# 5l1v3r1/PBS

Measured on AMD Instinct MI355X. Metric: co-run slowdown (%) vs solo + aggregate throughput, 4-tenant mix at 1/2/4/8 GPU, higher is better.
Workload: dtype bf16

## Files before the change

### csrc/hip/common.hpp

```cpp
#pragma once
#include <hip/hip_runtime.h>

#include <cstdint>
#include <cstdio>
#include <cstdlib>

namespace gpbs_hip {

constexpr int kXcds = 8;
constexpr int kMaxTenants = 64;
constexpr int kNumPmc = 4;
constexpr uint32_t kNoOwner = 0xFFFFFFFFu;
constexpr uint32_t kSplitBit = 0x80000000u;
constexpr uint32_t kOwnerMask = 0x7FFFFFFFu;

typedef __bf16 bf16x8 __attribute__((ext_vector_type(8)));
typedef float f32x4 __attribute__((ext_vector_type(4)));
typedef float f32x16 __attribute__((ext_vector_type(16)));
typedef unsigned int u32x4 __attribute__((ext_vector_type(4)));
typedef unsigned int u32x2 __attribute__((ext_vector_type(2)));
typedef unsigned short u16;
typedef unsigned int u32;
typedef unsigned long long u64;

__device__ __forceinline__ float bfl(u32 w) { return __uint_as_float(w << 16); }
__device__ __forceinline__ float bfh(u32 w) { return __uint_as_float(w & 0xffff0000u); }
__device__ __forceinline__ u32 pack2(float lo, float hi) {
  return (u32)__builtin_bit_cast(u16, (__bf16)lo) | ((u32)__builtin_bit_cast(u16, (__bf16)hi) << 16);
}

constexpr int kCtx = 4;
struct alignas(64) PartTable {
  u32 epoch;
  u32 flags;
  u32 hold;
  u32 pad0;
  union {
    u32 owner[kXcds * kCtx];
    u64 pair[kXcds][2];
  };
  u32 pad[12];
};
static_assert(sizeof(PartTable) == 192, "partition table layout");

struct alignas(64) WorkQueue {
  u32 next;
  u32 done;
  u32 exited;
  u32 stopped;
  u32 xnext[kXcds];
  u32 pad[4];
};

__device__ __forceinline__ void finish(WorkQueue* q, u32* status, u32 total) {
  if (threadIdx.x == 0) {
    asm volatile("s_waitcnt vmcnt(0)" ::: "memory");
    const u32 old = atomicAdd(&q->exited, 1u);
    if (old == gridDim.x - 1) {
      const u32 d = __hip_atomic_load(&q->done, __ATOMIC_RELAXED, __HIP_MEMORY_SCOPE_AGENT);
      if (status) __hip_atomic_store(status, d | 0x80000000u, __ATOMIC_RELAXED, __HIP_MEMORY_SCOPE_SYSTEM);
      __hip_atomic_store(&q->exited, 0u, __ATOMIC_RELAXED, __HIP_MEMORY_SCOPE_AGENT);
      __hip_atomic_store(&q->stopped, 0u, __ATOMIC_RELAXED, __HIP_MEMORY_SCOPE_AGENT);
      if (d >= total) {
        __hip_atomic_store(&q->next, 0u, __ATOMIC_RELAXED, __HIP_MEMORY_SCOPE_AGENT);
        __hip_atomic_store(&q->done, 0u, __ATOMIC_RELAXED, __HIP_MEMORY_SCOPE_AGENT);
#pragma unroll
        for (int x = 0; x < kXcds; ++x) __hip_atomic_store(&q->xnext[x], 0u, __ATOMIC_RELAXED, __HIP_MEMORY_SCOPE_AGENT);
      }
    }
  }
}


enum GateMode : u32 {
  GATE_NONE = 0, GATE_TABLE = 1, GATE_PARK = 2, GATE_DEVTABLE = 4, GATE_SPATIAL = 8,
  GATE_WAVEPRIO = 16,
  GATE_SE = 32,
  GATE_HOLD = 64,
};
constexpr u32 kParkSpins = 100;
constexpr u32 kHoldSpins = 256;

#define HIPCHECK(x)                                                                              \
  do {                                                                                           \
    hipError_t _e = (x);                                                                         \
    if (_e != hipSuccess) {                                                                      \
      fprintf(stderr, "[gpbs-hip] %s:%d %s -> %s\n", __FILE__, __LINE__, #x, hipGetErrorString(_e)); \
      return -(int)_e - 1000;                                                                    \
    }                                                                                            \
  } while (0)

__device__ __forceinline__ u32 xcc_id() {
  return __builtin_amdgcn_s_getreg((3 << 11) | (0 << 6) | 20);
}

__device__ __forceinline__ u32 hw_id() { return __builtin_amdgcn_s_getreg((31 << 11) | (0 << 6) | 4); }

__device__ __forceinline__ u32 cu_half() { return (hw_id() >> 14) & 1u; }

__device__ __forceinline__ u32 se_id() { return (hw_id() >> 13) & 3u; }

__device__ __forceinline__ u32 load_sys(const u32* p) {
  return __hip_atomic_load(p, __ATOMIC_RELAXED, __HIP_MEMORY_SCOPE_SYSTEM);
}

__device__ __forceinline__ void hold_wait(const PartTable* t, u32 mode) {
  if (!(mode & GATE_HOLD)) return;
  for (u32 k = 0; k < kHoldSpins; ++k) {
    const u32 h = (mode & GATE_DEVTABLE) ? __hip_atomic_load(&t->hold, __ATOMIC_RELAXED, __HIP_MEMORY_SCOPE_AGENT)
                                         : __hip_atomic_load(&t->hold, __ATOMIC_RELAXED, __HIP_MEMORY_SCOPE_SYSTEM);
    if (!h) return;
    __builtin_amdgcn_s_sleep(32);
  }
}

__device__ __forceinline__ bool owns(const PartTable* t, u32 mode, u32 me, u32 xcc) {
  if ((mode & 3) == GATE_NONE) return true;
  if (mode & GATE_SE) {
    const u32 se = se_id();
    const u32* w = t->owner + kCtx * (xcc & 7) + se;
    const u32 o = (mode & GATE_DEVTABLE) ? __hip_atomic_load(w, __ATOMIC_RELAXED, __HIP_MEMORY_SCOPE_AGENT)
                                         : __hip_atomic_load(w, __ATOMIC_RELAXED, __HIP_MEMORY_SCOPE_SYSTEM);
    return (o & kOwnerMask) == me;
  }
  const u64* q = t->pair[xcc & 7];
  const u64 p01 = (mode & GATE_DEVTABLE) ? __hip_atomic_load(q, __ATOMIC_RELAXED, __HIP_MEMORY_SCOPE_AGENT)
                                         : __hip_atomic_load(q, __ATOMIC_RELAXED, __HIP_MEMORY_SCOPE_SYSTEM);
  const u32 w0 = (u32)p01, w1 = (u32)(p01 >> 32);
  const bool h0 = (w0 & kOwnerMask) == me, h1 = (w1 & kOwnerMask) == me;
  if (!(mode & GATE_SPATIAL) || (h0 && h1)) {
    if (h0 || h1) return true;
    const u64 p23 = (mode & GATE_DEVTABLE) ? __hip_atomic_load(q + 1, __ATOMIC_RELAXED, __HIP_MEMORY_SCOPE_AGENT)
                                           : __hip_atomic_load(q + 1, __ATOMIC_RELAXED, __HIP_MEMORY_SCOPE_SYSTEM);
    return (u32)p23 == me || (u32)(p23 >> 32) == me;
  }
  if (h0) return !(w0 & kSplitBit) || cu_half() == 0;
  if (h1) return !(w1 & kSplitBit) || cu_half() == 1;
  return false;
}

__device__ __forceinline__ void count(u64* cnt, u32 me, u32 xcc, u64 inst, u64 cyc, u64 refs, u64 miss) {
  if (!cnt) return;
  u64* c = cnt + ((size_t)me * kXcds + (xcc & 7)) * kNumPmc;
  if (inst) __hip_atomic_fetch_add(c + 0, inst, __ATOMIC_RELAXED, __HIP_MEMORY_SCOPE_SYSTEM);
  if (cyc) __hip_atomic_fetch_add(c + 1, cyc, __ATOMIC_RELAXED, __HIP_MEMORY_SCOPE_SYSTEM);
  if (refs) __hip_atomic_fetch_add(c + 2, refs, __ATOMIC_RELAXED, __HIP_MEMORY_SCOPE_SYSTEM);
  if (miss) __hip_atomic_fetch_add(c + 3, miss, __ATOMIC_RELAXED, __HIP_MEMORY_SCOPE_SYSTEM);
}

__device__ __forceinline__ int grab_unit(WorkQueue* q, const PartTable* table, u32 mode, u32 me, u32 xcc,
                                         int* s_slot, u32 total) {
  if (threadIdx.x == 0) {
    int u = -1;
    hold_wait(table, mode);
    for (u32 spins = 0;; ++spins) {
      if (owns(table, mode, me, xcc)) {
        const u32 t = atomicAdd(&q->next, 1u);
        u = t < total ? (int)t : -1;
        break;
      }
      if ((mode & 3) != GATE_PARK || spins >= kParkSpins ||
          __hip_atomic_load(&q->next, __ATOMIC_RELAXED, __HIP_MEMORY_SCOPE_AGENT) >= total) {
        atomicAdd(&q->stopped, 1u);
        break;
      }
#pragma unroll
      for (int k = 0; k < 6; ++k) __builtin_amdgcn_s_sleep(127);
    }
    *s_slot = u;
  }
  __syncthreads();
  int u = *s_slot;
  __syncthreads();
  return u;
}


__device__ __forceinline__ void count_unit(u64* cnt, u32 me, u32 xcc, u64 inst, u64* t_last, u64 refs, u64 miss,
                                           WorkQueue* q) {
  if (threadIdx.x != 0) return;
  const u64 t = __builtin_amdgcn_s_memtime();
  count(cnt, me, xcc, inst, t - *t_last, refs, miss);
  *t_last = t;
  atomicAdd(&q->done, 1u);
}

}
```

### csrc/hip/fp8_gemm_kernels.hip

```cpp
#include "common.hpp"

namespace gpbs_fp8g {

using namespace gpbs_hip;

typedef int i32x8 __attribute__((ext_vector_type(8)));
typedef __attribute__((address_space(3))) char lds_t;

constexpr int FBM = 128, FBN = 128, FBK = 128, FNT = 256;
constexpr int kTile = FBM * FBK;
constexpr int kLds = 2 * 2 * kTile;
constexpr int kOne = 0x7f7f7f7f;

__device__ __forceinline__ void glds16(const void* g, lds_t* l) {
  __builtin_amdgcn_global_load_lds(g, (__attribute__((address_space(3))) void*)l, 16, 0, 0);
}

__device__ __forceinline__ u16 f2bf(float x) { return __builtin_bit_cast(u16, (__bf16)x); }

template <int BSHUF>
__global__ __launch_bounds__(FNT, 2) void k_gemm_fp8_tn(const unsigned char* __restrict__ A,
                                                        const float* __restrict__ sa,
                                                        const unsigned char* __restrict__ B,
                                                        const float* __restrict__ sb, u16* __restrict__ C, int M,
                                                        int N, int K, WorkQueue* q, const PartTable* table, u32 mode,
                                                        u32 me, u64* cnt, u32 inst_per_tile, u32 refs_per_tile,
                                                        u32 miss_per_tile, u32* status) {
  __shared__ __attribute__((aligned(16))) char smem[kLds + 16];
  lds_t* lds = (lds_t*)smem;
  int* s_slot = (int*)(smem + kLds);
  const u32 xcc = xcc_id();
  u64 t_last = __builtin_amdgcn_s_memtime();
  const int tid = threadIdx.x, lane = tid & 63, wid = tid >> 6;
  const int wr = wid >> 1, wc = wid & 1;
  const int tiles_m = (M + FBM - 1) / FBM, tiles_n = N / FBN, ntiles = tiles_m * tiles_n;
  const int nk = K / FBK;
  constexpr int GROUP_M = 8;

  int srow[4], schunk[4];
#pragma unroll
  for (int j = 0; j < 4; ++j) {
    srow[j] = 8 * (wid * 4 + j) + (lane >> 3);
    schunk[j] = (lane & 7) ^ (srow[j] & 7);
  }
  const int l16 = lane & 15, lq = lane >> 4;

  for (;;) {
    const int t = grab_unit(q, table, mode, me, xcc, s_slot, (u32)ntiles);
    if (t < 0) break;
    const int in_group = GROUP_M * tiles_n;
    const int g = t / in_group;
    const int first_m = g * GROUP_M;
    const int gsz = min(tiles_m - first_m, GROUP_M);
    const int tm = first_m + (t % in_group) % gsz;
    const int tn = (t % in_group) / gsz;

    size_t aoff[4], boff[4];
    int bstep;
#pragma unroll
    for (int j = 0; j < 4; ++j) {
      const int ra = min(tm * FBM + srow[j], M - 1);
      aoff[j] = (size_t)ra * K + schunk[j] * 16;
      if (BSHUF) {
        const int p = wid * 4 + j;
        boff[j] = (size_t)(tn * (FBN / 16) + (p >> 1)) * (K >> 8) * 4096 + (p & 1) * 1024 + lane * 16;
      } else {
        boff[j] = (size_t)(tn * FBN + srow[j]) * K + schunk[j] * 16;
      }
    }
    bstep = BSHUF ? 2048 : FBK;

    f32x4 acc[4][4];
#pragma unroll
    for (int i = 0; i < 4; ++i)
#pragma unroll
      for (int j = 0; j < 4; ++j) acc[i][j] = f32x4{0.f, 0.f, 0.f, 0.f};

    auto stage = [&](int buf, int kt) {
      lds_t* la = lds + buf * (2 * kTile);
      lds_t* lb = la + kTile;
#pragma unroll
      for (int j = 0; j < 4; ++j) {
        const int c = wid * 4 + j;
        glds16(A + aoff[j] + (size_t)kt * FBK, la + c * 1024);
        glds16(B + boff[j] + (size_t)kt * bstep, lb + c * 1024);
      }
    };
    auto frag = [&](const lds_t* img, int r0) -> i32x8 {
      const int r = r0 + l16;
      const lds_t* row = img + r * 128;
      const u32x4 lo = *(const __attribute__((address_space(3))) u32x4*)(row + (((2 * lq) ^ (r & 7)) << 4));
      const u32x4 hi = *(const __attribute__((address_space(3))) u32x4*)(row + (((2 * lq + 1) ^ (r & 7)) << 4));
      return i32x8{(int)lo[0], (int)lo[1], (int)lo[2], (int)lo[3], (int)hi[0], (int)hi[1], (int)hi[2], (int)hi[3]};
    };
    auto frag_shuf = [&](const lds_t* img, int r0) -> i32x8 {
      const lds_t* p = img + ((r0 >> 4) * 2 + (lq >> 1)) * 1024 + (lq & 1) * 512 + l16 * 16;
      const u32x4 lo = *(const __attribute__((address_space(3))) u32x4*)p;
      const u32x4 hi = *(const __attribute__((address_space(3))) u32x4*)(p + 256);
      return i32x8{(int)lo[0], (int)lo[1], (int)lo[2], (int)lo[3], (int)hi[0], (int)hi[1], (int)hi[2], (int)hi[3]};
    };

    stage(0, 0);
    asm volatile("s_waitcnt vmcnt(0)" ::: "memory");
    __syncthreads();
    int cur = 0;
    for (int kt = 0; kt < nk; ++kt) {
      if (kt + 1 < nk) stage(cur ^ 1, kt + 1);
      const lds_t* la = lds + cur * (2 * kTile);
      const lds_t* lb = la + kTile;
      i32x8 a[4], b[4];
#pragma unroll
      for (int i = 0; i < 4; ++i) {
        a[i] = frag(la, wr * 64 + i * 16);
        b[i] = BSHUF ? frag_shuf(lb, wc * 64 + i * 16) : frag(lb, wc * 64 + i * 16);
      }
#pragma unroll
      for (int i = 0; i < 4; ++i)
#pragma unroll
        for (int j = 0; j < 4; ++j)
          acc[i][j] = __builtin_amdgcn_mfma_scale_f32_16x16x128_f8f6f4(a[i], b[j], acc[i][j], 0, 0, 0, kOne, 0, kOne);
      asm volatile("s_waitcnt vmcnt(0)" ::: "memory");
      __syncthreads();
      cur ^= 1;
    }
#pragma unroll
    for (int j = 0; j < 4; ++j) {
      const int n = tn * FBN + wc * 64 + j * 16 + l16;
      const float wsc = sb[n];
#pragma unroll
      for (int i = 0; i < 4; ++i) {
        const int m = tm * FBM + wr * 64 + i * 16 + lq * 4;
#pragma unroll
        for (int r = 0; r < 4; ++r)
          if (m + r < M) C[(size_t)(m + r) * N + n] = f2bf((acc[i][j][r] * sa[m + r]) * wsc);
      }
    }
    count_unit(cnt, me, xcc, inst_per_tile, &t_last, refs_per_tile, miss_per_tile, q);
  }
  finish(q, status, (u32)ntiles);
}

}

using namespace gpbs_fp8g;

extern "C" {

int gpbs_hip_gemm_fp8_units(int M, int N) {
  if (M <= 0 || N <= 0 || N % FBN) return 0;
  return ((M + FBM - 1) / FBM) * (N / FBN);
}

int gpbs_hip_gemm_fp8(const void* Aq, const float* sa, const void* Bq, const float* sb, void* C, int M, int N, int K,
                      int b_shuffled, void* q, const void* table, unsigned mode, unsigned me, void* cnt, void* status,
                      int grid, hipStream_t s) {
  if (M <= 0 || N <= 0 || K <= 0 || N % FBN || K % FBK || (b_shuffled && K % 256)) return -22;
  const int ntiles = ((M + FBM - 1) / FBM) * (N / FBN);
  if (grid <= 0) grid = 256 * 2;
  if (grid > ntiles) grid = ntiles;
  const u32 inst = (u32)((K / FBK) * (64 + 32 + 64) + 64);
  const u32 refs = (u32)(((u64)(FBM + FBN) * K) / 128);
  const u32 miss = (u32)((((u64)M + N) * K / 128) / ntiles + (u64)FBM * FBN * 2 / 128);
  auto kern = b_shuffled ? k_gemm_fp8_tn<1> : k_gemm_fp8_tn<0>;
  hipLaunchKernelGGL(kern, dim3(grid), dim3(FNT), 0, s, (const unsigned char*)Aq, sa, (const unsigned char*)Bq, sb,
                     (u16*)C, M, N, K, (WorkQueue*)q, (const PartTable*)table, mode, me, (u64*)cnt, inst, refs, miss,
                     (u32*)status);
  return hipGetLastError() == hipSuccess ? 0 : -5;
}

}
```

### csrc/hip/tenant_kernels.hip

```cpp
#include "common.hpp"

namespace gpbs_hip {


__device__ __forceinline__ int grab_unit_x(WorkQueue* q, const PartTable* table, u32 mode, u32 me, u32 xcc,
                                           int* s_slot, u32 total) {
  if (threadIdx.x == 0) {
    int u = -1;
    hold_wait(table, mode);
    const u32 per = (total + kXcds - 1) / kXcds;
    for (u32 spins = 0;; ++spins) {
      if (owns(table, mode, me, xcc)) {
        for (u32 k = 0; k < (u32)kXcds; ++k) {
          const u32 r = (xcc + k) & (kXcds - 1);
          const u32 lo = r * per, hi = min(lo + per, total);
          if (lo >= hi) continue;
          if (__hip_atomic_load(&q->xnext[r], __ATOMIC_RELAXED, __HIP_MEMORY_SCOPE_AGENT) >= hi - lo) continue;
          const u32 t = atomicAdd(&q->xnext[r], 1u);
          if (t < hi - lo) {
            u = (int)(lo + t);
            atomicAdd(&q->next, 1u);
            break;
          }
        }
        break;
      }
      if ((mode & 3) != GATE_PARK || spins >= kParkSpins ||
          __hip_atomic_load(&q->next, __ATOMIC_RELAXED, __HIP_MEMORY_SCOPE_AGENT) >= total) {
        atomicAdd(&q->stopped, 1u);
        break;
      }
#pragma unroll
      for (int k = 0; k < 6; ++k) __builtin_amdgcn_s_sleep(127);
    }
    *s_slot = u;
  }
  __syncthreads();
  int u = *s_slot;
  __syncthreads();
  return u;
}


__device__ __forceinline__ u16 f2bf(float x) { return __builtin_bit_cast(u16, (__bf16)x); }
__device__ __forceinline__ float bf2f(u16 x) { return __uint_as_float(((u32)x) << 16); }

constexpr int GBM = 128, GBN = 128, GBK = 64, GNT = 256;
constexpr int kGemmLds = 2 * 2 * GBM * GBK * 2;

typedef __attribute__((address_space(3))) char lds_t;

__device__ __forceinline__ void glds16(const void* g, lds_t* l) {
  __builtin_amdgcn_global_load_lds(g, (__attribute__((address_space(3))) void*)l, 16, 0, 0);
}

__global__ __launch_bounds__(GNT, 2) void k_gemm_bf16_tn(const u16* __restrict__ A, const u16* __restrict__ Bt,
                                                         u16* __restrict__ C, int M, int N, int K, WorkQueue* q,
                                                         const PartTable* table, u32 mode, u32 me, u64* cnt,
                                                         u32 inst_per_tile, u32 refs_per_tile, u32 miss_per_tile,
                                                         u32* status) {
  __shared__ __attribute__((aligned(16))) char smem[kGemmLds + 16];
  lds_t* lds = (lds_t*)smem;
  int* s_slot = (int*)(smem + kGemmLds);
  const u32 xcc = xcc_id();
  u64 t_last = __builtin_amdgcn_s_memtime();
  const int tid = threadIdx.x, lane = tid & 63, wid = tid >> 6;
  const int wr = wid >> 1, wc = wid & 1;
  const int tiles_m = M / GBM, tiles_n = N / GBN, ntiles = tiles_m * tiles_n;
  const int nk = K / GBK;
  constexpr int GROUP_M = 8;

  int srow[4], scol[4];
#pragma unroll
  for (int j = 0; j < 4; ++j) {
    const int c = wid * 4 + j;
    srow[j] = 8 * c + (lane >> 3);
    scol[j] = (((lane & 7) ^ (srow[j] & 7)) * 8);
  }

  for (;;) {
    const int t = grab_unit(q, table, mode, me, xcc, s_slot, (u32)ntiles);
    if (t < 0) break;
    const int in_group = GROUP_M * tiles_n;
    const int g = t / in_group;
    const int first_m = g * GROUP_M;
    const int gsz = min(tiles_m - first_m, GROUP_M);
    const int tm = first_m + (t % in_group) % gsz;
    const int tn = (t % in_group) / gsz;
    const u16* Ab = A + (size_t)tm * GBM * K;
    const u16* Bb = Bt + (size_t)tn * GBN * K;

    f32x4 acc[4][4];
#pragma unroll
    for (int i = 0; i < 4; ++i)
#pragma unroll
      for (int j = 0; j < 4; ++j) acc[i][j] = f32x4{0.f, 0.f, 0.f, 0.f};

    auto stage = [&](int buf, int kt) {
      lds_t* la = lds + buf * (2 * GBM * GBK * 2);
      lds_t* lb = la + GBM * GBK * 2;
#pragma unroll
      for (int j = 0; j < 4; ++j) {
        const int c = wid * 4 + j;
        glds16(Ab + (size_t)srow[j] * K + kt * GBK + scol[j], la + c * 1024);
        glds16(Bb + (size_t)srow[j] * K + kt * GBK + scol[j], lb + c * 1024);
      }
    };

    stage(0, 0);
    asm volatile("s_waitcnt vmcnt(0)" ::: "memory");
    __syncthreads();
    int cur = 0;
    for (int kt = 0; kt < nk; ++kt) {
      if (kt + 1 < nk) stage(cur ^ 1, kt + 1);
      const lds_t* la = lds + cur * (2 * GBM * GBK * 2);
      const lds_t* lb = la + GBM * GBK * 2;
#pragma unroll
      for (int s = 0; s < 2; ++s) {
        bf16x8 a[4], b[4];
        const int chunk = s * 4 + (lane >> 4);
#pragma unroll
        for (int i = 0; i < 4; ++i) {
          const int ra = wr * 64 + i * 16 + (lane & 15);
          a[i] = *(const __attribute__((address_space(3))) bf16x8*)(la + ra * 128 + ((chunk ^ (ra & 7)) << 4));
          const int rb = wc * 64 + i * 16 + (lane & 15);
          b[i] = *(const __attribute__((address_space(3))) bf16x8*)(lb + rb * 128 + ((chunk ^ (rb & 7)) << 4));
        }
#pragma unroll
        for (int i = 0; i < 4; ++i)
#pragma unroll
          for (int j = 0; j < 4; ++j) acc[i][j] = __builtin_amdgcn_mfma_f32_16x16x32_bf16(a[i], b[j], acc[i][j], 0, 0, 0);
      }
      asm volatile("s_waitcnt vmcnt(0)" ::: "memory");
      __syncthreads();
      cur ^= 1;
    }
#pragma unroll
    for (int i = 0; i < 4; ++i)
#pragma unroll
      for (int j = 0; j < 4; ++j) {
        const int m = tm * GBM + wr * 64 + i * 16 + (lane >> 4) * 4;
        const int n = tn * GBN + wc * 64 + j * 16 + (lane & 15);
#pragma unroll
        for (int r = 0; r < 4; ++r) C[(size_t)(m + r) * N + n] = f2bf(acc[i][j][r]);
      }
    count_unit(cnt, me, xcc, inst_per_tile, &t_last, refs_per_tile, miss_per_tile, q);
  }
  finish(q, status, (u32)ntiles);
}

constexpr int G2_BM = 256, G2_BK = 64, G2_NT = 512;
constexpr u32 kGemmXRange = 1u << 16;
constexpr u32 kGemmBlock2D = 1u << 17;
constexpr u32 kGemmStatic = 1u << 18;
constexpr int kGemmOptsLive = 1 | 8 | 1 << 23;
constexpr int kGemmOptsShipped = 256 | 8192 | 65536 | 131072;
static int g_gemm_opts = 8;
constexpr int kG2Half = 128 * 128;
constexpr int kG2Buf = 4 * kG2Half;
constexpr int kG2Lds = 2 * kG2Buf;

__device__ __forceinline__ int g2_swz(int r) { return (r >> 1) & 7; }

__global__ __launch_bounds__(G2_NT, 1) void k_gemm256_bf16_tn(const u16* __restrict__ A, const u16* __restrict__ Bt,
                                                             u16* __restrict__ C, int M, int N, int K, WorkQueue* q,
                                                             const PartTable* table, u32 mode, u32 me, u64* cnt,
                                                             u32 inst_per_tile, u32 refs_per_tile, u32 miss_per_tile,
                                                             u32* status) {
  __shared__ __attribute__((aligned(16))) char smem[kG2Lds + 16];
  lds_t* lds = (lds_t*)smem;
  int* s_slot = (int*)(smem + kG2Lds);
  const u32 xcc = xcc_id();
  u64 t_last = __builtin_amdgcn_s_memtime();
  const int tid = threadIdx.x, lane = tid & 63, wid = tid >> 6;
  const int wu = __builtin_amdgcn_readfirstlane(wid);
  const int wr = wu >> 2, wc = wu & 3;
  const int tiles_m = M / G2_BM, tiles_n = N / G2_BM, ntiles = tiles_m * tiles_n;
  const int nt = K / G2_BK;
  int soff[2];
#pragma unroll
  for (int j = 0; j < 2; ++j) {
    const int row = 8 * (2 * wid + j) + (lane >> 3);
    soff[j] = row * K + (((lane & 7) ^ g2_swz(row)) * 8);
  }
  int soffa[4];
#pragma unroll
  for (int j = 0; j < 4; ++j) {
    const int row = 8 * (4 * (wid & 3) + j) + (lane >> 3);
    soffa[j] = row * K + (((lane & 7) ^ g2_swz(row)) * 8);
  }
  const int l16 = lane & 15, lq = lane >> 4;
  const int bh = wc >> 1, bc = (wc & 1) * 64;
  int units_seen = 0;

  for (;;) {
    const int tile = (mode & kGemmStatic) ? (units_seen ? -1 : (int)blockIdx.x)
                     : (mode & kGemmXRange) ? grab_unit_x(q, table, mode, me, xcc, s_slot, (u32)ntiles)
                                            : grab_unit(q, table, mode, me, xcc, s_slot, (u32)ntiles);
    if (tile < 0) break;
    int tm = tile / tiles_n, tn = tile % tiles_n;
    if ((mode & kGemmBlock2D) && (tiles_m & 3) == 0 && (tiles_n & 1) == 0 && ntiles % kXcds == 0) {
      const int per = ntiles / kXcds;
      const int bm = tiles_m / 4, bn = tiles_n / 2;
      const int g = (mode & kGemmXRange) ? tile / per : tile % kXcds;
      const int jj = (mode & kGemmXRange) ? tile % per : tile / kXcds;
      tm = (g >> 1) * bm + jj / bn;
      tn = (g & 1) * bn + jj % bn;
    }
    const u16* Ab = A + (size_t)tm * G2_BM * K;
    const u16* Bb = Bt + (size_t)tn * G2_BM * K;
    auto stage = [&](int kind, int h, int t) {
      const u16* src = (kind ? Bb : Ab) + (size_t)h * 128 * K + t * G2_BK;
      lds_t* dst = lds + (t & 1) * kG2Buf + (kind * 2 + h) * kG2Half + wid * 2048;
      glds16(src + soff[0], dst);
      glds16(src + soff[1], dst + 1024);
    };
    auto stage_own_a = [&](int t) {
      const u16* src = Ab + (size_t)wr * 128 * K + t * G2_BK;
      lds_t* dst = lds + (t & 1) * kG2Buf + wr * kG2Half + (wid & 3) * 4096;
#pragma unroll
      for (int j = 0; j < 4; ++j) glds16(src + soffa[j], dst + j * 1024);
    };
    auto frag = [&](int b, int kind, int h, int r0, int s) -> bf16x8 {
      const int r = r0 + l16;
      const lds_t* p = lds + b * kG2Buf + (kind * 2 + h) * kG2Half + r * 128 + (((4 * s + lq) ^ g2_swz(r)) << 4);
      return *(const __attribute__((address_space(3))) bf16x8*)p;
    };
    f32x4 acc[8][4];
#pragma unroll
    for (int i = 0; i < 8; ++i)
#pragma unroll
      for (int j = 0; j < 4; ++j) acc[i][j] = f32x4{0.f, 0.f, 0.f, 0.f};
    stage(1, 0, 0); stage(1, 1, 0); stage(0, 0, 0); stage(0, 1, 0);
    asm volatile("s_waitcnt vmcnt(0)" ::: "memory");
    __builtin_amdgcn_s_barrier();
    if (wr == 1) __builtin_amdgcn_s_barrier();
    bf16x8 a[4][2], b[4][2];
    for (int t = 0; t < nt; ++t) {
      const int buf = t & 1;
      const bool more = t + 1 < nt;
#pragma unroll
      for (int j = 0; j < 4; ++j)
#pragma unroll
        for (int s2 = 0; s2 < 2; ++s2) b[j][s2] = frag(buf, 1, bh, bc + j * 16, s2);
      __builtin_amdgcn_sched_barrier(0);
#pragma unroll
      for (int i = 0; i < 4; ++i)
#pragma unroll
        for (int s2 = 0; s2 < 2; ++s2) a[i][s2] = frag(buf, 0, wr, i * 16, s2);
      if (more) {
        stage(1, 0, t + 1); stage(1, 1, t + 1);
      } else {
        asm volatile("s_waitcnt vmcnt(0)" ::: "memory");
      }
      __builtin_amdgcn_s_barrier();
      asm volatile("s_waitcnt lgkmcnt(0)" ::: "memory");
      __builtin_amdgcn_s_setprio(1);
#pragma unroll
      for (int s2 = 0; s2 < 2; ++s2)
#pragma unroll
        for (int i = 0; i < 4; ++i)
#pragma unroll
          for (int j = 0; j < 4; ++j)
            acc[i][j] = __builtin_amdgcn_mfma_f32_16x16x32_bf16(b[j][s2], a[i][s2], acc[i][j], 0, 0, 0);
      __builtin_amdgcn_s_setprio(0);
      __builtin_amdgcn_s_barrier();
#pragma unroll
      for (int i = 0; i < 4; ++i)
#pragma unroll
        for (int s2 = 0; s2 < 2; ++s2) a[i][s2] = frag(buf, 0, wr, 64 + i * 16, s2);
      if (more) {
        stage_own_a(t + 1);
        asm volatile("s_waitcnt vmcnt(4)" ::: "memory");
      }
      __builtin_amdgcn_s_barrier();
      asm volatile("s_waitcnt lgkmcnt(0)" ::: "memory");
      __builtin_amdgcn_s_setprio(1);
#pragma unroll
      for (int s2 = 0; s2 < 2; ++s2)
#pragma unroll
        for (int i = 0; i < 4; ++i)
#pragma unroll
          for (int j = 0; j < 4; ++j)
            acc[4 + i][j] = __builtin_amdgcn_mfma_f32_16x16x32_bf16(b[j][s2], a[i][s2], acc[4 + i][j], 0, 0, 0);
      __builtin_amdgcn_s_setprio(0);
      asm volatile("s_waitcnt vmcnt(0)" ::: "memory");
      __builtin_amdgcn_s_barrier();
    }
    if (wr == 0) __builtin_amdgcn_s_barrier();
#pragma unroll
    for (int i = 0; i < 8; ++i)
#pragma unroll
      for (int j = 0; j < 4; ++j) {
        const int m = wr * 128 + i * 16 + l16;
        const int c8 = wc * 16 + j * 4 + lq;
        const u32 lo = (u32)f2bf(acc[i][j][0]) | ((u32)f2bf(acc[i][j][1]) << 16);
        const u32 hi = (u32)f2bf(acc[i][j][2]) | ((u32)f2bf(acc[i][j][3]) << 16);
        *(__attribute__((address_space(3))) u32x2*)(lds + m * 512 + ((c8 ^ (m & 15)) << 3)) = u32x2{lo, hi};
      }
    __syncthreads();
#pragma unroll
    for (int p = 0; p < 16; ++p) {
      const int row = p * 16 + (tid >> 5), c16 = tid & 31;
      u32x4 v = *(const __attribute__((address_space(3))) u32x4*)(lds + row * 512 + (((2 * c16) ^ (row & 14)) << 3));
      if (row & 1) v = u32x4{v.z, v.w, v.x, v.y};
      u32x4* dst = (u32x4*)(C + (size_t)(tm * G2_BM + row) * N + tn * G2_BM + c16 * 8);
      __builtin_nontemporal_store(v, dst);
    }
    __syncthreads();
    ++units_seen;
    if (!(mode & kGemmStatic)) count_unit(cnt, me, xcc, inst_per_tile, &t_last, refs_per_tile, miss_per_tile, q);
  }
  if (!(mode & kGemmStatic)) finish(q, status, (u32)ntiles);
}

constexpr int SNT = 256, SUNROLL = 16, RUNROLL = 6;

template <int U, bool NTS>
__global__ __launch_bounds__(SNT) void k_stream_copy(const f32x4* __restrict__ src, f32x4* __restrict__ dst,
                                                    u64 n4, u32 chunk4, WorkQueue* q, const PartTable* table, u32 mode,
                                                    u32 me, u64* cnt, u32* status) {
  __shared__ int s_slot[4];
  const u32 xcc = xcc_id();
  u64 t_last = __builtin_amdgcn_s_memtime();
  const u32 nchunks = (u32)((n4 + chunk4 - 1) / chunk4);
  const u64 lines = (u64)chunk4 * 16 / 128;
  const u64 inst = (u64)chunk4 * 2 / 64 + 8;
  for (;;) {
    const int c = grab_unit(q, table, mode, me, xcc, s_slot, nchunks);
    if (c < 0) break;
    const u64 base = (u64)c * chunk4;
    const u64 end = min(base + chunk4, n4);
    for (u64 i = base + threadIdx.x; i < end; i += (u64)SNT * U) {
      f32x4 v[U];
#pragma unroll
      for (int k = 0; k < U; ++k) {
        const u64 idx = i + (u64)k * SNT;
        if (idx < end) v[k] = __builtin_nontemporal_load(src + idx);
      }
#pragma unroll
      for (int k = 0; k < U; ++k) {
        const u64 idx = i + (u64)k * SNT;
        if (idx < end) {
          if constexpr (NTS)
            __builtin_nontemporal_store(v[k], dst + idx);
          else
            dst[idx] = v[k];
        }
      }
    }
    count_unit(cnt, me, xcc, inst, &t_last, 2 * lines, 2 * lines, q);
  }
  finish(q, status, nchunks);
}

template <int NT, int U, bool NTL, bool NTS>
__global__ __launch_bounds__(NT) void k_reduce_bf16(const u32x4* __restrict__ a, const u32x4* __restrict__ b,
                                                    u32x4* __restrict__ out, u64 n8, u32 chunk8, WorkQueue* q,
                                                    const PartTable* table, u32 mode, u32 me, u64* cnt,
                                                    u32* status) {
  __shared__ int s_slot[4];
  const u32 xcc = xcc_id();
  u64 t_last = __builtin_amdgcn_s_memtime();
  const u32 nchunks = (u32)((n8 + chunk8 - 1) / chunk8);
  const u64 lines = (u64)chunk8 * 16 / 128;
  const u64 inst = (u64)chunk8 * 3 / 64 + (u64)chunk8 * 16 / 64;
  for (;;) {
    const int c = grab_unit(q, table, mode, me, xcc, s_slot, nchunks);
    if (c < 0) break;
    const u64 base = (u64)c * chunk8, end = min(base + chunk8, n8);
    for (u64 i = base + threadIdx.x; i < end; i += (u64)NT * U) {
      u32x4 x[U], y[U];
#pragma unroll
      for (int k = 0; k < U; ++k) {
        const u64 idx = i + (u64)k * NT;
        if (idx < end) {
          if constexpr (NTL) {
            x[k] = __builtin_nontemporal_load(a + idx);
            y[k] = __builtin_nontemporal_load(b + idx);
          } else {
            x[k] = a[idx];
            y[k] = b[idx];
          }
        }
      }
#pragma unroll
      for (int k = 0; k < U; ++k) {
        const u64 idx = i + (u64)k * NT;
        if (idx >= end) continue;
        const u32* px = (const u32*)&x[k];
        const u32* py = (const u32*)&y[k];
        u32x4 r;
        u32* pr = (u32*)&r;
#pragma unroll
        for (int w = 0; w < 4; ++w) {
          const float lo = bf2f((u16)(px[w] & 0xffff)) + bf2f((u16)(py[w] & 0xffff));
          const float hi = bf2f((u16)(px[w] >> 16)) + bf2f((u16)(py[w] >> 16));
          pr[w] = (u32)f2bf(lo) | ((u32)f2bf(hi) << 16);
        }
        if constexpr (NTS)
          __builtin_nontemporal_store(r, out + idx);
        else
          out[idx] = r;
      }
    }
    count_unit(cnt, me, xcc, inst, &t_last, 3 * lines, 3 * lines, q);
  }
  finish(q, status, nchunks);
}

constexpr int GV_U = 2;

__device__ __forceinline__ float dot8(const u32x4 w, const u32x4 v) {
  float s = 0.f;
#pragma unroll
  for (int e = 0; e < 4; ++e) {
    s += __uint_as_float(w[e] << 16) * __uint_as_float(v[e] << 16);
    s += __uint_as_float(w[e] & 0xffff0000u) * __uint_as_float(v[e] & 0xffff0000u);
  }
  return s;
}

__global__ __launch_bounds__(256) __attribute__((amdgpu_waves_per_eu(5, 8))) void k_gemv_bf16(const u16* __restrict__ W, const u16* __restrict__ x,
                                                  float* __restrict__ y, int R, int K, WorkQueue* q,
                                                  const PartTable* table, u32 mode, u32 me, u64* cnt,
                                                  u32* status) {
  __shared__ int s_slot[4];
  if (mode & GATE_WAVEPRIO) __builtin_amdgcn_s_setprio(3);
  const u32 xcc = xcc_id();
  u64 t_last = __builtin_amdgcn_s_memtime();
  const int lane = threadIdx.x & 63, wid = threadIdx.x >> 6;
  const u32 nchunks = (u32)((R + 15) / 16);
  const u64 lines = (u64)16 * K * 2 / 128;
  const int nk = K / 512;
  const u32x4* xv = (const u32x4*)x;
  for (;;) {
    const int c = grab_unit(q, table, mode, me, xcc, s_slot, nchunks);
    if (c < 0) break;
    const int row0 = c * 16 + wid * 4;
    const u32x4* wr[4];
#pragma unroll
    for (int r = 0; r < 4; ++r) wr[r] = (const u32x4*)(W + (size_t)min(row0 + r, R - 1) * K);
    float acc[4] = {0.f, 0.f, 0.f, 0.f};
    int kc = 0;
    for (; kc + GV_U <= nk; kc += GV_U) {
      u32x4 xr[GV_U], wv[GV_U][4];
#pragma unroll
      for (int u = 0; u < GV_U; ++u) {
        const int k = (kc + u) * 64 + lane;
        xr[u] = xv[k];
#pragma unroll
        for (int r = 0; r < 4; ++r) wv[u][r] = __builtin_nontemporal_load(wr[r] + k);
      }
#pragma unroll
      for (int u = 0; u < GV_U; ++u)
#pragma unroll
        for (int r = 0; r < 4; ++r) acc[r] += dot8(wv[u][r], xr[u]);
    }
    for (; kc < nk; ++kc) {
      const int k = kc * 64 + lane;
      const u32x4 xr = xv[k];
#pragma unroll
      for (int r = 0; r < 4; ++r) acc[r] += dot8(__builtin_nontemporal_load(wr[r] + k), xr);
    }
#pragma unroll
    for (int r = 0; r < 4; ++r) {
      float s = acc[r];
#pragma unroll
      for (int off = 32; off > 0; off >>= 1) s += __shfl_xor(s, off, 64);
      if (lane == 0 && row0 + r < R) y[row0 + r] = s;
    }
    count_unit(cnt, me, xcc, (u64)16 * (K / 512 + 8), &t_last, lines, lines, q);
  }
  finish(q, status, nchunks);
}

__global__ void k_census(u32* out, const PartTable* table, u32 mode, u32 me) {
  const u32 xcc = xcc_id();
  const bool ok = owns(table, mode, me, xcc);
  if (threadIdx.x == 0) {
    out[blockIdx.x * 4 + 0] = xcc;
    out[blockIdx.x * 4 + 1] = hw_id();
    out[blockIdx.x * 4 + 2] = ok ? 1u : 0u;
    out[blockIdx.x * 4 + 3] = 0xC0FFEEu;
  }
  if (ok) {
    u64 t = __builtin_amdgcn_s_memtime();
    while (__builtin_amdgcn_s_memtime() - t < 2000) __builtin_amdgcn_s_sleep(1);
  }
}

}

using namespace gpbs_hip;

extern "C" {

int gpbs_hip_set_gemm_opts(int opts) {
  const int old = g_gemm_opts;
  if (opts < 0) return old;
  const int gone = opts & ~(kGemmOptsLive | kGemmOptsShipped);
  static bool warned = false;
  if (gone && !warned) {
    warned = true;
    fprintf(stderr,
            "gpbs_hip_set_gemm_opts: bits 0x%x select GEMM variants that were removed (docs/gemm_lab.md); "
            "the shipped schedule runs\n",
            gone);
  }
  g_gemm_opts = opts & kGemmOptsLive;
  return old;
}

int gpbs_hip_gemm_units(int M, int N) {
  if (M % G2_BM == 0 && N % G2_BM == 0) return (M / G2_BM) * (N / G2_BM);
  return (M / GBM) * (N / GBN);
}

int gpbs_hip_gemm_bf16(const void* A, const void* Bt, void* C, int M, int N, int K, void* q, const void* table,
                       unsigned mode, unsigned me, void* cnt, void* status, int grid, hipStream_t s) {
  if (M % GBM || N % GBN || K % GBK || M <= 0 || N <= 0 || K <= 0) return -22;
  if (M % G2_BM == 0 && N % G2_BM == 0) {
    const int ntiles = (M / G2_BM) * (N / G2_BM);
    if (grid <= 0) grid = 256;
    if (grid > ntiles) grid = ntiles;
    const u32 inst = (u32)((G2_BM / 16) * (G2_BM / 16) * (K / 32) + (K / G2_BK) * 64 + 128);
    const u32 refs = (u32)(((u64)2 * G2_BM * K * 2) / 128);
    const u32 miss = (u32)((((u64)M + N) * K * 2 / 128) / ntiles + (u64)G2_BM * G2_BM * 2 / 128);
    const u32 m2 = mode | ((g_gemm_opts & 1) ? kGemmXRange : 0u) |
                   ((g_gemm_opts & 8) && ntiles % kXcds == 0 ? kGemmBlock2D : 0u) |
                   ((g_gemm_opts & (1 << 23)) && (mode & 3) == GATE_NONE && grid == ntiles ? kGemmStatic : 0u);
    hipLaunchKernelGGL(k_gemm256_bf16_tn, dim3(grid), dim3(G2_NT), 0, s, (const u16*)A, (const u16*)Bt, (u16*)C, M, N,
                       K, (WorkQueue*)q, (const PartTable*)table, m2, me, (u64*)cnt, inst, refs, miss, (u32*)status);
    return hipGetLastError() == hipSuccess ? 0 : -5;
  }
  const int ntiles = (M / GBM) * (N / GBN);
  if (grid <= 0) grid = 256 * 2;
  if (grid > ntiles) grid = ntiles;
  const u32 inst = (u32)((GBM / 16) * (GBN / 16) * (K / 32) * 2 + (K / GBK) * 32 + 64);
  const u32 refs = (u32)(((u64)(GBM + GBN) * K * 2) / 128);
  const u32 miss = (u32)((((u64)M + N) * K * 2 / 128) / ntiles + (u64)GBM * GBN * 2 / 128);
  hipLaunchKernelGGL(k_gemm_bf16_tn, dim3(grid), dim3(GNT), 0, s, (const u16*)A, (const u16*)Bt, (u16*)C, M, N, K,
                     (WorkQueue*)q, (const PartTable*)table, mode, me, (u64*)cnt, inst, refs, miss, (u32*)status);
  return hipGetLastError() == hipSuccess ? 0 : -5;
}

static int g_stream_opts = 0;

int gpbs_hip_set_stream_opts(int opts) {
  const int old = g_stream_opts;
  if (opts >= 0) g_stream_opts = opts;
  return old;
}

int gpbs_hip_stream_copy(const void* src, void* dst, unsigned long long bytes, unsigned chunk_bytes, void* q,
                         const void* table, unsigned mode, unsigned me, void* cnt, void* status, int grid, hipStream_t s) {
  if (bytes % 16 || chunk_bytes % 16 || chunk_bytes == 0) return -22;
  if (grid <= 0) grid = 256;
  using K = void (*)(const f32x4*, f32x4*, u64, u32, WorkQueue*, const PartTable*, u32, u32, u64*, u32*);
  static const K tab[4] = {k_stream_copy<SUNROLL, true>, k_stream_copy<SUNROLL, false>, k_stream_copy<8, true>,
                           k_stream_copy<8, false>};
  hipLaunchKernelGGL(tab[g_stream_opts & 3], dim3(grid), dim3(SNT), 0, s, (const f32x4*)src, (f32x4*)dst, bytes / 16,
                     chunk_bytes / 16, (WorkQueue*)q, (const PartTable*)table, mode, me, (u64*)cnt, (u32*)status);
  return hipGetLastError() == hipSuccess ? 0 : -5;
}

static int g_reduce_opts = 8;

int gpbs_hip_set_reduce_opts(int opts) {
  const int old = g_reduce_opts;
  if (opts >= 0) g_reduce_opts = opts;
  return old;
}

int gpbs_hip_reduce_bf16(const void* a, const void* b, void* out, unsigned long long bytes, unsigned chunk_bytes,
                         void* q, const void* table, unsigned mode, unsigned me, void* cnt, void* status, int grid, hipStream_t s) {
  if (bytes % 16 || chunk_bytes % 16 || chunk_bytes == 0) return -22;
  if (grid <= 0) grid = 256;
  using K = void (*)(const u32x4*, const u32x4*, u32x4*, u64, u32, WorkQueue*, const PartTable*, u32, u32, u64*, u32*);
#define RV(NT, U) {k_reduce_bf16<NT, U, true, true>, k_reduce_bf16<NT, U, false, true>, \
                   k_reduce_bf16<NT, U, true, false>, k_reduce_bf16<NT, U, false, false>}
  static const K table256[4][4] = {RV(256, 6), RV(256, 8), RV(256, 4), RV(256, 12)};
  static const K table512[4][4] = {RV(512, 6), RV(512, 8), RV(512, 4), RV(512, 12)};
#undef RV
  const int o = g_reduce_opts;
  const int nt = (o & 16) ? 512 : 256;
  const K kern = ((o & 16) ? table512 : table256)[o & 3][((o >> 2) & 1) | (((o >> 3) & 1) << 1)];
  hipLaunchKernelGGL(kern, dim3(grid), dim3(nt), 0, s, (const u32x4*)a, (const u32x4*)b, (u32x4*)out,
                     bytes / 16, chunk_bytes / 16, (WorkQueue*)q, (const PartTable*)table, mode, me, (u64*)cnt, (u32*)status);
  return hipGetLastError() == hipSuccess ? 0 : -5;
}

int gpbs_hip_gemv_bf16(const void* W, const void* x, void* y, int R, int K, void* q, const void* table, unsigned mode,
                       unsigned me, void* cnt, void* status, int grid, hipStream_t s) {
  if (K % 512 || R <= 0) return -22;
  if (grid <= 0) grid = (R + 15) / 16;
  if (grid > 256) grid = 256;
  hipLaunchKernelGGL(k_gemv_bf16, dim3(grid), dim3(256), 0, s, (const u16*)W, (const u16*)x, (float*)y, R, K,
                     (WorkQueue*)q, (const PartTable*)table, mode, me, (u64*)cnt, (u32*)status);
  return hipGetLastError() == hipSuccess ? 0 : -5;
}

int gpbs_hip_census(void* out, int blocks, const void* table, unsigned mode, unsigned me, hipStream_t s) {
  hipLaunchKernelGGL(k_census, dim3(blocks), dim3(64), 0, s, (u32*)out, (const PartTable*)table, mode, me);
  return hipGetLastError() == hipSuccess ? 0 : -5;
}

}
```

Before: 1.277.

## Overlap next-tile grab and prefetch with epilogue; batch per-block completion counting

Each block now counts its completed units locally and adds them to a packed 64-bit exit/done word once at finish, which replaces a global atomic increment per unit. In the persistent GEMM, the ticket for the next tile (or the ownership words) is fetched during the last k-iteration. The next tile's first stage loads are issued between the two halves of the C store. This hides queue latency and pipeline fill behind the epilogue, at the cost of more complex control flow and register pressure. The done counter semantics also change: progress is visible only at block exit.

```diff
diff --git a/csrc/hip/common.hpp b/csrc/hip/common.hpp
--- a/csrc/hip/common.hpp
+++ b/csrc/hip/common.hpp
@@ -1,6 +1,7 @@
 #pragma once
 #include <hip/hip_runtime.h>
 
+#include <cstddef>
 #include <cstdint>
 #include <cstdio>
 #include <cstdlib>
@@ -49,24 +50,24 @@
   u32 exited;
   u32 stopped;
   u32 xnext[kXcds];
-  u32 pad[4];
-};
-
-__device__ __forceinline__ void finish(WorkQueue* q, u32* status, u32 total) {
+  u64 exitw;
+  u32 pad[2];
+};
+static_assert(sizeof(WorkQueue) == 64 && offsetof(WorkQueue, exitw) == 48, "work queue layout");
+
+__device__ __forceinline__ void finish(WorkQueue* q, u32* status, u32 total, u32 units) {
   if (threadIdx.x == 0) {
-    asm volatile("s_waitcnt vmcnt(0)" ::: "memory");
-    const u32 old = atomicAdd(&q->exited, 1u);
-    if (old == gridDim.x - 1) {
-      const u32 d = __hip_atomic_load(&q->done, __ATOMIC_RELAXED, __HIP_MEMORY_SCOPE_AGENT);
+    const u64 old = __hip_atomic_fetch_add(&q->exitw, ((u64)1 << 32) | units, __ATOMIC_RELAXED, __HIP_MEMORY_SCOPE_AGENT);
+    if ((u32)(old >> 32) == gridDim.x - 1) {
+      const u32 d = (u32)old + units;
       if (status) __hip_atomic_store(status, d | 0x80000000u, __ATOMIC_RELAXED, __HIP_MEMORY_SCOPE_SYSTEM);
-      __hip_atomic_store(&q->exited, 0u, __ATOMIC_RELAXED, __HIP_MEMORY_SCOPE_AGENT);
       __hip_atomic_store(&q->stopped, 0u, __ATOMIC_RELAXED, __HIP_MEMORY_SCOPE_AGENT);
       if (d >= total) {
         __hip_atomic_store(&q->next, 0u, __ATOMIC_RELAXED, __HIP_MEMORY_SCOPE_AGENT);
-        __hip_atomic_store(&q->done, 0u, __ATOMIC_RELAXED, __HIP_MEMORY_SCOPE_AGENT);
 #pragma unroll
         for (int x = 0; x < kXcds; ++x) __hip_atomic_store(&q->xnext[x], 0u, __ATOMIC_RELAXED, __HIP_MEMORY_SCOPE_AGENT);
       }
+      __hip_atomic_store(&q->exitw, d >= total ? (u64)0 : (u64)d, __ATOMIC_RELAXED, __HIP_MEMORY_SCOPE_AGENT);
     }
   }
 }
@@ -134,6 +135,34 @@
                                            : __hip_atomic_load(q + 1, __ATOMIC_RELAXED, __HIP_MEMORY_SCOPE_SYSTEM);
     return (u32)p23 == me || (u32)(p23 >> 32) == me;
   }
+  if (h0) return !(w0 & kSplitBit) || cu_half() == 0;
+  if (h1) return !(w1 & kSplitBit) || cu_half() == 1;
+  return false;
+}
+
+struct OwnWords {
+  u64 p01, p23;
+};
+__device__ __forceinline__ OwnWords own_load(const PartTable* t, u32 mode, u32 xcc) {
+  const u64* q = t->pair[xcc & 7];
+  OwnWords w;
+  if (mode & GATE_DEVTABLE) {
+    w.p01 = __hip_atomic_load(q, __ATOMIC_RELAXED, __HIP_MEMORY_SCOPE_AGENT);
+    w.p23 = __hip_atomic_load(q + 1, __ATOMIC_RELAXED, __HIP_MEMORY_SCOPE_AGENT);
+  } else {
+    w.p01 = __hip_atomic_load(q, __ATOMIC_RELAXED, __HIP_MEMORY_SCOPE_SYSTEM);
+    w.p23 = __hip_atomic_load(q + 1, __ATOMIC_RELAXED, __HIP_MEMORY_SCOPE_SYSTEM);
+  }
+  return w;
+}
+__device__ __forceinline__ bool own_eval(const OwnWords w, u32 mode, u32 me) {
+  const u32 w0 = (u32)w.p01, w1 = (u32)(w.p01 >> 32), w2 = (u32)w.p23, w3 = (u32)(w.p23 >> 32);
+  if (mode & GATE_SE) {
+    const u32 se = se_id();
+    return ((se & 2 ? (se & 1 ? w3 : w2) : (se & 1 ? w1 : w0)) & kOwnerMask) == me;
+  }
+  const bool h0 = (w0 & kOwnerMask) == me, h1 = (w1 & kOwnerMask) == me;
+  if (!(mode & GATE_SPATIAL) || (h0 && h1)) return h0 || h1 || w2 == me || w3 == me;
   if (h0) return !(w0 & kSplitBit) || cu_half() == 0;
   if (h1) return !(w1 & kSplitBit) || cu_half() == 1;
   return false;
@@ -175,6 +204,12 @@
   return u;
 }
 
+__device__ __forceinline__ u32 take_ticket(WorkQueue* q) {
+  u32 zero = 0;
+  asm volatile("" : "+v"(zero));
+  return atomicAdd(&q->next + zero, 1u);
+}
+
 
 __device__ __forceinline__ void count_unit(u64* cnt, u32 me, u32 xcc, u64 inst, u64* t_last, u64 refs, u64 miss,
                                            WorkQueue* q) {
@@ -185,4 +220,13 @@
   atomicAdd(&q->done, 1u);
 }
 
-}
+__device__ __forceinline__ void tally_unit(u64* cnt, u32 me, u32 xcc, u64 inst, u64* t_last, u64 refs, u64 miss,
+                                           u32* units) {
+  ++*units;
+  if (threadIdx.x != 0) return;
+  const u64 t = __builtin_amdgcn_s_memtime();
+  count(cnt, me, xcc, inst, t - *t_last, refs, miss);
+  *t_last = t;
+}
+
+}
diff --git a/csrc/hip/fp8_gemm_kernels.hip b/csrc/hip/fp8_gemm_kernels.hip
--- a/csrc/hip/fp8_gemm_kernels.hip
+++ b/csrc/hip/fp8_gemm_kernels.hip
@@ -31,6 +31,7 @@
   int* s_slot = (int*)(smem + kLds);
   const u32 xcc = xcc_id();
   u64 t_last = __builtin_amdgcn_s_memtime();
+  u32 units = 0;
   const int tid = threadIdx.x, lane = tid & 63, wid = tid >> 6;
   const int wr = wid >> 1, wc = wid & 1;
   const int tiles_m = (M + FBM - 1) / FBM, tiles_n = N / FBN, ntiles = tiles_m * tiles_n;
@@ -135,9 +136,9 @@
           if (m + r < M) C[(size_t)(m + r) * N + n] = f2bf((acc[i][j][r] * sa[m + r]) * wsc);
       }
     }
-    count_unit(cnt, me, xcc, inst_per_tile, &t_last, refs_per_tile, miss_per_tile, q);
+    tally_unit(cnt, me, xcc, inst_per_tile, &t_last, refs_per_tile, miss_per_tile, &units);
   }
-  finish(q, status, (u32)ntiles);
+  finish(q, status, (u32)ntiles, units);
 }
 
 }
diff --git a/csrc/hip/tenant_kernels.hip b/csrc/hip/tenant_kernels.hip
--- a/csrc/hip/tenant_kernels.hip
+++ b/csrc/hip/tenant_kernels.hip
@@ -1,3 +1,5 @@
+#include <type_traits>
+
 #include "common.hpp"
 
 namespace gpbs_hip {
@@ -64,6 +66,7 @@
   int* s_slot = (int*)(smem + kGemmLds);
   const u32 xcc = xcc_id();
   u64 t_last = __builtin_amdgcn_s_memtime();
+  u32 units = 0;
   const int tid = threadIdx.x, lane = tid & 63, wid = tid >> 6;
   const int wr = wid >> 1, wc = wid & 1;
   const int tiles_m = M / GBM, tiles_n = N / GBN, ntiles = tiles_m * tiles_n;
@@ -144,9 +147,9 @@
 #pragma unroll
         for (int r = 0; r < 4; ++r) C[(size_t)(m + r) * N + n] = f2bf(acc[i][j][r]);
       }
-    count_unit(cnt, me, xcc, inst_per_tile, &t_last, refs_per_tile, miss_per_tile, q);
-  }
-  finish(q, status, (u32)ntiles);
+    tally_unit(cnt, me, xcc, inst_per_tile, &t_last, refs_per_tile, miss_per_tile, &units);
+  }
+  finish(q, status, (u32)ntiles, units);
 }
 
 constexpr int G2_BM = 256, G2_BK = 64, G2_NT = 512;
@@ -183,22 +186,17 @@
     const int row = 8 * (2 * wid + j) + (lane >> 3);
     soff[j] = row * K + (((lane & 7) ^ g2_swz(row)) * 8);
   }
-  int soffa[4];
-#pragma unroll
-  for (int j = 0; j < 4; ++j) {
-    const int row = 8 * (4 * (wid & 3) + j) + (lane >> 3);
-    soffa[j] = row * K + (((lane & 7) ^ g2_swz(row)) * 8);
-  }
   const int l16 = lane & 15, lq = lane >> 4;
   const int bh = wc >> 1, bc = (wc & 1) * 64;
-  int units_seen = 0;
-
-  for (;;) {
-    const int tile = (mode & kGemmStatic) ? (units_seen ? -1 : (int)blockIdx.x)
-                     : (mode & kGemmXRange) ? grab_unit_x(q, table, mode, me, xcc, s_slot, (u32)ntiles)
-                                            : grab_unit(q, table, mode, me, xcc, s_slot, (u32)ntiles);
-    if (tile < 0) break;
-    int tm = tile / tiles_n, tn = tile % tiles_n;
+  u32 units = 0;
+  const bool early = !(mode & (kGemmStatic | kGemmXRange | GATE_HOLD));
+  const bool gated = (mode & 3) != GATE_NONE;
+  constexpr int kNoTile = -1, kGrabLate = -2;
+
+  const u16 *Ab = nullptr, *Bb = nullptr;
+  int tm = 0, tn = 0;
+  auto locate = [&](int tile) {
+    tm = tile / tiles_n, tn = tile % tiles_n;
     if ((mode & kGemmBlock2D) && (tiles_m & 3) == 0 && (tiles_n & 1) == 0 && ntiles % kXcds == 0) {
       const int per = ntiles / kXcds;
       const int bm = tiles_m / 4, bn = tiles_n / 2;
@@ -207,8 +205,29 @@
       tm = (g >> 1) * bm + jj / bn;
       tn = (g & 1) * bn + jj % bn;
     }
-    const u16* Ab = A + (size_t)tm * G2_BM * K;
-    const u16* Bb = Bt + (size_t)tn * G2_BM * K;
+    Ab = A + (size_t)tm * G2_BM * K;
+    Bb = Bt + (size_t)tn * G2_BM * K;
+  };
+
+  int tile = (mode & kGemmStatic) ? (int)blockIdx.x : kGrabLate;
+  bool staged = false;
+  for (;;) {
+    if (tile == kGrabLate)
+      tile = (mode & kGemmXRange) ? grab_unit_x(q, table, mode, me, xcc, s_slot, (u32)ntiles)
+                                  : grab_unit(q, table, mode, me, xcc, s_slot, (u32)ntiles);
+    if (tile < 0) break;
+    if (!staged) locate(tile);
+    u16* Cb = C + (size_t)tm * G2_BM * N + tn * G2_BM;
+    int soffa[4];
+    {
+      int tid_s = tid;
+      asm volatile("" : "+v"(tid_s));
+#pragma unroll
+      for (int j = 0; j < 4; ++j) {
+        const int row = 8 * (4 * ((tid_s >> 6) & 3) + j) + ((tid_s & 63) >> 3);
+        soffa[j] = row * K + (((tid_s & 7) ^ g2_swz(row)) * 8);
+      }
+    }
     auto stage = [&](int kind, int h, int t) {
       const u16* src = (kind ? Bb : Ab) + (size_t)h * 128 * K + t * G2_BK;
       lds_t* dst = lds + (t & 1) * kG2Buf + (kind * 2 + h) * kG2Half + wid * 2048;
@@ -231,14 +250,18 @@
     for (int i = 0; i < 8; ++i)
 #pragma unroll
       for (int j = 0; j < 4; ++j) acc[i][j] = f32x4{0.f, 0.f, 0.f, 0.f};
-    stage(1, 0, 0); stage(1, 1, 0); stage(0, 0, 0); stage(0, 1, 0);
+    if (!staged) {
+      stage(1, 0, 0); stage(1, 1, 0); stage(0, 0, 0); stage(0, 1, 0);
+    }
     asm volatile("s_waitcnt vmcnt(0)" ::: "memory");
     __builtin_amdgcn_s_barrier();
     if (wr == 1) __builtin_amdgcn_s_barrier();
     bf16x8 a[4][2], b[4][2];
-    for (int t = 0; t < nt; ++t) {
+    u32 ticket, ticket_g;
+    OwnWords ow;
+    auto ktile = [&](const int t, auto more_c) {
+      constexpr bool more = decltype(more_c)::value;
       const int buf = t & 1;
-      const bool more = t + 1 < nt;
 #pragma unroll
       for (int j = 0; j < 4; ++j)
 #pragma unroll
@@ -248,10 +271,12 @@
       for (int i = 0; i < 4; ++i)
 #pragma unroll
         for (int s2 = 0; s2 < 2; ++s2) a[i][s2] = frag(buf, 0, wr, i * 16, s2);
-      if (more) {
+      if constexpr (more) {
         stage(1, 0, t + 1); stage(1, 1, t + 1);
       } else {
         asm volatile("s_waitcnt vmcnt(0)" ::: "memory");
+        if (early && !gated && tid == 0) ticket = take_ticket(q);
+        if (early && gated && tid == 0) ow = own_load(table, mode, xcc);
       }
       __builtin_amdgcn_s_barrier();
       asm volatile("s_waitcnt lgkmcnt(0)" ::: "memory");
@@ -269,7 +294,7 @@
       for (int i = 0; i < 4; ++i)
 #pragma unroll
         for (int s2 = 0; s2 < 2; ++s2) a[i][s2] = frag(buf, 0, wr, 64 + i * 16, s2);
-      if (more) {
+      if constexpr (more) {
         stage_own_a(t + 1);
         asm volatile("s_waitcnt vmcnt(4)" ::: "memory");
       }
@@ -286,32 +311,59 @@
       __builtin_amdgcn_s_setprio(0);
       asm volatile("s_waitcnt vmcnt(0)" ::: "memory");
       __builtin_amdgcn_s_barrier();
+    };
+    for (int t = 0; t + 1 < nt; ++t) ktile(t, std::true_type{});
+    ktile(nt - 1, std::false_type{});
+    bool got = early && !gated;
+    if (early && gated && tid == 0) {
+      got = own_eval(ow, mode, me);
+      if (got) ticket_g = take_ticket(q);
     }
     if (wr == 0) __builtin_amdgcn_s_barrier();
+    int tid_e = tid;
+    asm volatile("" : "+v"(tid_e));
+    const int l16e = tid_e & 15, lqe = (tid_e >> 4) & 3;
 #pragma unroll
     for (int i = 0; i < 8; ++i)
 #pragma unroll
       for (int j = 0; j < 4; ++j) {
-        const int m = wr * 128 + i * 16 + l16;
-        const int c8 = wc * 16 + j * 4 + lq;
+        const int m = wr * 128 + i * 16 + l16e;
+        const int c8 = wc * 16 + j * 4 + lqe;
         const u32 lo = (u32)f2bf(acc[i][j][0]) | ((u32)f2bf(acc[i][j][1]) << 16);
         const u32 hi = (u32)f2bf(acc[i][j][2]) | ((u32)f2bf(acc[i][j][3]) << 16);
         *(__attribute__((address_space(3))) u32x2*)(lds + m * 512 + ((c8 ^ (m & 15)) << 3)) = u32x2{lo, hi};
       }
+    if (tid == 0) {
+      const u32 tk = gated ? ticket_g : ticket;
+      *s_slot = (mode & kGemmStatic) ? kNoTile : !got ? kGrabLate : tk < (u32)ntiles ? (int)tk : kNoTile;
+    }
     __syncthreads();
-#pragma unroll
-    for (int p = 0; p < 16; ++p) {
-      const int row = p * 16 + (tid >> 5), c16 = tid & 31;
-      u32x4 v = *(const __attribute__((address_space(3))) u32x4*)(lds + row * 512 + (((2 * c16) ^ (row & 14)) << 3));
-      if (row & 1) v = u32x4{v.z, v.w, v.x, v.y};
-      u32x4* dst = (u32x4*)(C + (size_t)(tm * G2_BM + row) * N + tn * G2_BM + c16 * 8);
-      __builtin_nontemporal_store(v, dst);
-    }
-    __syncthreads();
-    ++units_seen;
-    if (!(mode & kGemmStatic)) count_unit(cnt, me, xcc, inst_per_tile, &t_last, refs_per_tile, miss_per_tile, q);
-  }
-  if (!(mode & kGemmStatic)) finish(q, status, (u32)ntiles);
+    int next = *s_slot;
+    auto store_rows = [&](int p0) {
+      const int r0 = tid_e >> 5, c16 = tid_e & 31;
+      const lds_t* src = lds + (p0 * 16 + r0) * 512 + (((2 * c16) ^ (r0 & 14)) << 3);
+      u32x4* dst = (u32x4*)(Cb + (size_t)(p0 * 16 + r0) * N + c16 * 8);
+#pragma unroll
+      for (int p = 0; p < 8; ++p) {
+        u32x4 v = *(const __attribute__((address_space(3))) u32x4*)(src + p * 16 * 512);
+        if (r0 & 1) v = u32x4{v.z, v.w, v.x, v.y};
+        __builtin_nontemporal_store(v, dst);
+        dst += 2 * (size_t)N;
+      }
+    };
+    store_rows(0);
+    asm volatile("s_waitcnt lgkmcnt(0)" ::: "memory");
+    __builtin_amdgcn_s_barrier();
+    staged = next >= 0;
+    if (staged) {
+      locate(next);
+      stage(1, 0, 0); stage(1, 1, 0); stage(0, 0, 0); stage(0, 1, 0);
+    }
+    store_rows(8);
+    if (!(mode & kGemmStatic)) tally_unit(cnt, me, xcc, inst_per_tile, &t_last, refs_per_tile, miss_per_tile, &units);
+    tile = next;
+  }
+  if (!(mode & kGemmStatic)) finish(q, status, (u32)ntiles, units);
 }
 
 constexpr int SNT = 256, SUNROLL = 16, RUNROLL = 6;
@@ -323,6 +375,7 @@
   __shared__ int s_slot[4];
   const u32 xcc = xcc_id();
   u64 t_last = __builtin_amdgcn_s_memtime();
+  u32 units = 0;
   const u32 nchunks = (u32)((n4 + chunk4 - 1) / chunk4);
   const u64 lines = (u64)chunk4 * 16 / 128;
   const u64 inst = (u64)chunk4 * 2 / 64 + 8;
@@ -349,9 +402,9 @@
         }
       }
     }
-    count_unit(cnt, me, xcc, inst, &t_last, 2 * lines, 2 * lines, q);
-  }
-  finish(q, status, nchunks);
+    tally_unit(cnt, me, xcc, inst, &t_last, 2 * lines, 2 * lines, &units);
+  }
+  finish(q, status, nchunks, units);
 }
 
 template <int NT, int U, bool NTL, bool NTS>
@@ -362,6 +415,7 @@
   __shared__ int s_slot[4];
   const u32 xcc = xcc_id();
   u64 t_last = __builtin_amdgcn_s_memtime();
+  u32 units = 0;
   const u32 nchunks = (u32)((n8 + chunk8 - 1) / chunk8);
   const u64 lines = (u64)chunk8 * 16 / 128;
   const u64 inst = (u64)chunk8 * 3 / 64 + (u64)chunk8 * 16 / 64;
@@ -404,9 +458,9 @@
           out[idx] = r;
       }
     }
-    count_unit(cnt, me, xcc, inst, &t_last, 3 * lines, 3 * lines, q);
-  }
-  finish(q, status, nchunks);
+    tally_unit(cnt, me, xcc, inst, &t_last, 3 * lines, 3 * lines, &units);
+  }
+  finish(q, status, nchunks, units);
 }
 
 constexpr int GV_U = 2;
@@ -429,6 +483,7 @@
   if (mode & GATE_WAVEPRIO) __builtin_amdgcn_s_setprio(3);
   const u32 xcc = xcc_id();
   u64 t_last = __builtin_amdgcn_s_memtime();
+  u32 units = 0;
   const int lane = threadIdx.x & 63, wid = threadIdx.x >> 6;
   const u32 nchunks = (u32)((R + 15) / 16);
   const u64 lines = (u64)16 * K * 2 / 128;
@@ -470,9 +525,9 @@
       for (int off = 32; off > 0; off >>= 1) s += __shfl_xor(s, off, 64);
       if (lane == 0 && row0 + r < R) y[row0 + r] = s;
     }
-    count_unit(cnt, me, xcc, (u64)16 * (K / 512 + 8), &t_last, lines, lines, q);
-  }
-  finish(q, status, nchunks);
+    tally_unit(cnt, me, xcc, (u64)16 * (K / 512 + 8), &t_last, lines, lines, &units);
+  }
+  finish(q, status, nchunks, units);
 }
 
 __global__ void k_census(u32* out, const PartTable* table, u32 mode, u32 me) {
```

Result: slower. 1.256 (-1.6%).
